# svip-lab/impersonator

Measured on AMD Instinct MI355X. Metric: frames/sec (256x256 motion-imitation, batch=8), higher is better.
Workload: dtype bf16x3; 1 GPU; Imitator inference 256x256 batch=8, random-init ImpersonatorGenerator + synthetic SMPL, 1 source; frames=1024, batch_per_gpu=8, image_size=256, parallelism=frame-sharded replicas x1, grid_sample_align_corners=False, lanes=2, batches_per_launch_sequence=4, frames_per_launch=32, precision=bf16x3, precision_policy=auto

## Files before the change

impersonator_amd/csrc/conv.hip:

```cpp
#include <type_traits>

#include "conv.h"
#include "split.h"
#include "sample.h"

namespace lwg {
namespace {

typedef float f32x16 __attribute__((ext_vector_type(16)));
#pragma clang diagnostic ignored "-Winline-asm"

constexpr int BM = kConvBM;
constexpr int BK = kConvBK;
constexpr int LDK = BK + 4;

template <int BN, int WM, int WN, bool WIDE = false, int NWAVES = 4, int BMT = BM, int TC2 = 0>
__device__ __forceinline__ void igemm_epilogue(const ConvArgs &a, const ConvPhase &ph, int phase, f32x16 (&acc)[WM][WN],
                                               float *smem, int tid, int lane, int wave_m, int wave_n, int img, int rem0, int n0,
                                               int mtile, int sub_stride = 0)
{
    unsigned ones = ~0u;
    asm volatile("" : "+s"(ones));
    lane = (int)__builtin_amdgcn_mbcnt_hi(ones, __builtin_amdgcn_mbcnt_lo(ones, 0u));
    tid = (wave_m * (BN / (32 * WN)) + wave_n) * 64 + lane;
// ... 843 lines not shown
        for (int i = 0; i < WM; ++i)
#pragma unroll
            for (int j = 0; j < WN; ++j)
#pragma unroll
                for (int r = 0; r < 16; ++r) keep += acc[i][j][r];
        if (keep == 123.456f) a.y[0] = 1.f;
    }
    __syncthreads();
    }
}

template <int NHW, int B_CH, int Q, int QB, int NS, int HT = 7>
struct HaloSched {
    static constexpr int nh(int t) { return t < HT ? NHW / HT + (t < NHW % HT ? 1 : 0) : 0; }
    static constexpr int tap_of(int k) { int t = 0; while (hstart(t + 1) <= k) ++t; return t; }
    static constexpr bool dma_at(int t, int q) { for (int p = 0; p < lps(t); ++p) if (pos(t, p) == q) return true; return false; }
    static constexpr int nfree(int t, int q0) { int n = 0; for (int q = q0; q < QB; ++q) n += dma_at(t, q) ? 0 : 1; return n; }
    static constexpr int conv_first(int nconv, int nslot, int slot, int piece) { return conv_range(nconv, nslot, slot, piece) / 16; }
    static constexpr int conv_last(int nconv, int nslot, int slot, int piece) { return conv_range(nconv, nslot, slot, piece) % 16; }
    static constexpr int conv_range(int nconv, int nslot, int slot, int piece) {
        if (nconv == 1) {
            if (piece != 0) return 0;
            if (nslot >= 7)
                return slot == 0 ? 0 * 16 + 1 : slot == 3 ? 1 * 16 + 3 : slot == 4 ? 3 * 16 + 5 : slot == 5 ? 5 * 16 + 7 : slot == 6 ? 7 * 16 + 8 : 0;
            return slot == 0 ? 0 * 16 + 1 : slot == 2 ? 1 * 16 + 4 : slot == 3 ? 4 * 16 + 6 : slot == 4 ? 6 * 16 + 8 : 0;
        }
        if (nslot >= 8) {
            if (slot >= 8 || (slot & 1) != piece) return 0;
            return (slot >> 1) == 0 ? 0 * 16 + 1 : (slot >> 1) == 1 ? 1 * 16 + 3 : (slot >> 1) == 2 ? 3 * 16 + 5 : 5 * 16 + 8;
        }
// ... 9 lines not shown
    }
    static constexpr int hstart(int t) { int n = 0; for (int u = 0; u < t; ++u) n += nh(u); return n; }
    static constexpr int lps(int t) { return nh(t) + B_CH; }
    static constexpr int pos(int t, int p) { return (p + 1) * Q / lps(t) - 1; }
    static constexpr int issued(int t) { int n = 0; for (int p = 0; p < lps(t); ++p) n += pos(t, p) < QB ? 1 : 0; return n; }
    static constexpr int nwait(int t) { int n = issued(t); for (int d = 1; d <= NS - 3; ++d) n += lps((t + 9 - d) % 9); return n; }
};

struct HaloCT {
    static constexpr int phase(int t) { return t == 0 ? 0 : t < 3 ? 1 : t < 5 ? 2 : 3; }
    static constexpr int tap(int t) { return t == 0 ? 0 : t < 3 ? t - 1 : t < 5 ? t - 3 : t - 5; }
    static constexpr int dy(int t) { return (t == 4 || t == 7 || t == 8) ? 1 : 0; }
    static constexpr int dx(int t) { return (t == 2 || t == 6 || t == 8) ? 1 : 0; }
};

template <int BN, int WM, int WN, int NS, int TC, int BMT = BM, int CT = 0, bool RAW = false>
__global__ __launch_bounds__(64 * (BMT / (32 * WM)) * (BN / (32 * WN))) void conv3x3_halo_bf16x3(const ConvArgs a)
{
    constexpr int NPH = CT ? 4 : 1, PADL = CT ? 0 : 1;
    constexpr int WAVES_N = BN / (32 * WN), WAVES_M = BMT / (32 * WM), NW = WAVES_M * WAVES_N;
    static_assert((NW == 4 || NW == 8) && (NS == 3 || NS == 4) && BMT % TC == 0 && TC % 32 == 0, "layout");
    constexpr int TR = BMT / TC, HC = TC + 2 - (CT ? 1 : 0), HR = TR + 2 - (CT ? 1 : 0), HP = HR * HC;
    constexpr int NCH = (HP + 7) / 8;
    constexpr int NHW = (NCH + NW - 1) / NW;
    constexpr int HALO = NCH * 8 * BK;
    constexpr int B_CH = BN / 8 / NW, BSTAGE = BN * BK, BOFF = 2 * HALO;
    static_assert(B_CH >= 1, "a weight chunk per wave");
    constexpr int TILES = WM * WN, Q = 6 * TILES, QB = Q * 3 / 4, NL = 2 * (WM + WN);
    constexpr int RPM = (NL + (Q - QB) - 1) / (Q - QB);
    constexpr int HT = RAW ? 6 : 7;
    using S = HaloSched<NHW, B_CH, Q, QB, NS, HT>;
    static_assert(S::hstart(9) == NHW && Q >= NHW / HT + 1 + B_CH, "halo pieces fit their taps, one piece per MFMA at most");
    static_assert(!RAW || (NW % 2 == 0 && S::tap_of(NHW - 1) + 3 <= 8), "RAW: chunk parity per wave, conversions end ahead of the barrier of tap 8");
    constexpr int DUMMY = BOFF + NS * BSTAGE;
    constexpr int SSOFF = DUMMY + 8 * BK;

    extern __shared__ __attribute__((aligned(16))) float smem[];
    const int tid = threadIdx.x, lane = tid & 63;
    const int wave = __builtin_amdgcn_readfirstlane(tid >> 6);
    const int wave_m = wave / WAVES_N, wave_n = wave % WAVES_N;
    unsigned long long tr_t0 = 0, tr_rt0 = 0, tr_loop0 = 0, tr_loop1 = 0;
    if (a.trace) {
        tr_t0 = __builtin_amdgcn_s_memtime();
        tr_rt0 = __builtin_amdgcn_s_memrealtime();
    }
    int bx = blockIdx.x;
    const int by = blockIdx.y;
    if (!a.natural_order && (gridDim.x & 7) == 0) bx = (blockIdx.x & 7) * (gridDim.x >> 3) + (blockIdx.x >> 3);
// ... 12 lines not shown
    };
    auto dma16 = [&](unsigned voff, const char *sbase, unsigned lds_byte) {
        asm volatile("s_mov_b32 m0, %2\n\t"
                     "s_nop 0\n\t"
                     "global_load_lds_dwordx4 %0, %1"
                     :
                     : "v"(voff), "s"(sbase), "s"(lds_byte)
                     : "memory", "m0");
    };
    const ConvPhase ph = a.ph[0];
    const int lr = lane >> 3, ls = lane & 7;
    const float *xin = a.x + (size_t)img * a.H * a.W * a.ldx;
    const char *x_base = uniform_ptr(xin);
    const unsigned zoff_b = (unsigned)((const char *)a.zeros - (const char *)xin);

    unsigned hoff[NHW];
    unsigned inside = 0;
#pragma unroll
    for (int j = 0; j < NHW; ++j) {
        int c = wave + NW * j;
        if (c >= NCH) c -= NCH;
        const int p = c * 8 + lr;
        const int hr = p / HC, hc = p - hr * HC;
        const int gh = h0 - PADL + hr, gw = w0 - PADL + hc;
        const bool ok = p < HP && (unsigned)gh < (unsigned)a.H && (unsigned)gw < (unsigned)a.W;
        hoff[j] = ok ? (unsigned)(((gh * a.W + gw) * a.ldx + (ls ^ ((p >> 1) & 7)) * 4) * 4) : zoff_b;
        if (RAW && ok && wave + NW * j < NCH) inside |= 1u << j;
    }
    unsigned wvoff[NPH][B_CH];
#pragma unroll
    for (int pp = 0; pp < NPH; ++pp)
#pragma unroll
        for (int j = 0; j < B_CH; ++j) {
            const int row = (wave * B_CH + j) * 8 + lr;
            wvoff[pp][j] = (unsigned)(((n0 + row) * a.ph[pp].Kpad + (ls ^ ((row >> 1) & 7)) * 4) * 4);
        }
    const char *w_phase[NPH];
#pragma unroll
    for (int pp = 0; pp < NPH; ++pp) w_phase[pp] = uniform_ptr(a.w_split + a.ph[pp].w_off);
    const unsigned cin4 = (unsigned)a.Cin * 4u;
    const int nslices = a.Cin / BK;
    const unsigned wave_b = __builtin_amdgcn_readfirstlane(lds_base + (unsigned)((BOFF + wave * B_CH * 8 * BK) * 4));

    auto halo_piece = [&](int j, int sl, int hs) {
        int c = wave + NW * j;
        unsigned dst = (unsigned)((hs * HALO + c * 8 * BK) * 4);
        if (c >= NCH) {
            c -= NCH;
            dst = RAW ? (unsigned)(DUMMY * 4) : (unsigned)((hs * HALO + c * 8 * BK) * 4);
        }
        dma16(hoff[j], x_base + __builtin_amdgcn_readfirstlane((unsigned)sl * (BK * 4u)), __builtin_amdgcn_readfirstlane(lds_base + dst));
    };
    [[maybe_unused]] float4 ssa = {0.f, 0.f, 0.f, 0.f}, ssb = {0.f, 0.f, 0.f, 0.f};
    [[maybe_unused]] auto load_ss = [&](int sl) {
        const int g = ls ^ ((((wave & 1) << 2) + (lr >> 1)) & 7);
        const float *q = smem + SSOFF + (sl * BK - a.raw_from + 4 * g) * 2;
        ssa = *reinterpret_cast<const float4 *>(q);
        ssb = *reinterpret_cast<const float4 *>(q + 4);
    };
    [[maybe_unused]] const int cv_swz = (((wave & 1) << 2) + (lr >> 1)) & 7, cv_g = ls ^ cv_swz;
    [[maybe_unused]] const int cv_rd = lr * 128 + ls * 16;
    [[maybe_unused]] const int cv_hi = lr * 128 + (((cv_g >> 1) ^ cv_swz) << 4) + ((cv_g & 1) << 3);
    [[maybe_unused]] const int cv_lo = lr * 128 + (((4 + (cv_g >> 1)) ^ cv_swz) << 4) + ((cv_g & 1) << 3);
    [[maybe_unused]] const int cv_dummy = DUMMY * 4 + lane * 16;
    struct Conv { float4 v, y, hf; bf16x4_t h, l; int ahi, alo; };
    [[maybe_unused]] Conv cvA, cvB;
    [[maybe_unused]] auto convert_step = [&](int j, Conv &c, int hs, int step, bool live) {
// ... 11 lines not shown
            c.h[0] = (__bf16)c.y.x; c.h[1] = (__bf16)c.y.y; c.h[2] = (__bf16)c.y.z; c.h[3] = (__bf16)c.y.w;
        } else if (step == 4) {
            c.hf = make_float4((float)c.h[0], (float)c.h[1], (float)c.h[2], (float)c.h[3]);
        } else if (step == 5) {
            c.l[0] = (__bf16)(c.y.x - c.hf.x); c.l[1] = (__bf16)(c.y.y - c.hf.y);
            c.l[2] = (__bf16)(c.y.z - c.hf.z); c.l[3] = (__bf16)(c.y.w - c.hf.w);
        } else if (step == 6) {
            c.ahi = live ? chunk + cv_hi : cv_dummy;
            c.alo = live ? chunk + cv_lo : cv_dummy + 8;
        } else {
            *reinterpret_cast<bf16x4_t *>(base + c.ahi) = c.h;
            *reinterpret_cast<bf16x4_t *>(base + c.alo) = c.l;
        }
    };
    auto weight_piece = [&](int jb, int it, int is, int slot) {
        const int pp = CT ? HaloCT::phase(it) : 0, ti = CT ? HaloCT::tap(it) : it;
        dma16(wvoff[pp][jb], w_phase[pp] + __builtin_amdgcn_readfirstlane((unsigned)ti * cin4 + (unsigned)is * (BK * 4u)),
              __builtin_amdgcn_readfirstlane(wave_b + (unsigned)((slot * BSTAGE + jb * 8 * BK) * 4)));
    };

    f32x16 acc[NPH][WM][WN];
#pragma unroll
    for (int pp = 0; pp < NPH; ++pp)
#pragma unroll
        for (int i = 0; i < WM; ++i)
#pragma unroll
            for (int j = 0; j < WN; ++j)
#pragma unroll
                for (int r = 0; r < 16; ++r) acc[pp][i][j][r] = 0.f;

    const int frow = lane & 31, half = lane >> 5, fsw = (frow >> 1) & 7;
    int pl[WM];
#pragma unroll
    for (int i = 0; i < WM; ++i) {
        const int m = wave_m * 32 * WM + i * 32;
        pl[i] = (m / TC) * HC + (m % TC) + frow;
    }
    auto a_addr = [&](int i, int tap, int hs) {
        const int p = pl[i] + (CT ? HaloCT::dy(tap) * HC + HaloCT::dx(tap) : (tap / 3) * HC + (tap % 3));
        return hs * (HALO * 4) + p * 128 + ((half ^ ((p >> 1) & 7)) << 4);
    };
    const int b_row = (wave_n * 32 * WN + frow) * BK;
    int fcol[4];
#pragma unroll
    for (int c = 0; c < 4; ++c) fcol[c] = (((2 * c + half) ^ fsw) * 4);
    struct Frags { float4 ah[WM], al[WM], bh[WN], bl[WN]; };
    const char *smem_b = reinterpret_cast<const char *>(smem);
    auto load_one = [&](const int (&aa)[WM], int bslot, int kb, Frags &f, int idx) {
        const float *Bs = smem + BOFF + bslot * BSTAGE + b_row;
        if (idx < WM) f.al[idx] = *reinterpret_cast<const float4 *>(smem_b + (aa[idx] ^ (64 + 32 * kb)));
        else if (idx < WM + WN) f.bh[idx - WM] = *reinterpret_cast<const float4 *>(Bs + (idx - WM) * 32 * BK + fcol[kb]);
        else if (idx < 2 * WM + WN) f.ah[idx - WM - WN] = *reinterpret_cast<const float4 *>(smem_b + (aa[idx - WM - WN] ^ (32 * kb)));
        else f.bl[idx - 2 * WM - WN] = *reinterpret_cast<const float4 *>(Bs + (idx - 2 * WM - WN) * 32 * BK + fcol[2 + kb]);
    };
    Frags fr;
    int cur_a[WM];

    auto stage_body = [&](auto tap_c, auto issue_c, int sl, int slot) {
        constexpr int T = decltype(tap_c)::value;
        constexpr bool ISSUE = decltype(issue_c)::value;
        constexpr int TN = (T + 1) % 9;
        constexpr int IT = (T + NS - 1) % 9;
        const int slot1 = slot + 1 == NS ? 0 : slot + 1;
        const int slot2 = slot == 0 ? NS - 1 : slot - 1;
        const int hs = sl & 1, hs_next = T == 8 ? hs ^ 1 : hs;
        const int is = sl + (T + NS - 1 >= 9 ? 1 : 0);
        const int sl_halo = sl + 1 < nslices ? sl + 1 : 0;
        Frags f1, nx;
        int nxt_a[WM];
        [[maybe_unused]] const bool raw_next = RAW && sl + 1 < nslices && (sl + 1) * BK >= a.raw_from;
        [[maybe_unused]] const unsigned live_bits = raw_next ? inside : 0u;
        if constexpr (RAW) {
            if (T == S::tap_of(0) + 3) load_ss(sl + 1 < nslices ? sl + 1 : 0);
        }
#pragma unroll
        for (int q = 0; q < Q; ++q) {
            const int kb = q / (3 * TILES), r = q % (3 * TILES);
            const int t = r / TILES, i = (r / WN) % WM, j = r % WN;
            if (q == QB) {
                __builtin_amdgcn_sched_barrier(0);
                if (ISSUE) {
                    asm volatile("s_waitcnt vmcnt(%0) lgkmcnt(0)" ::"n"(S::nwait(T)) : "memory");
                } else {
                    asm volatile("s_waitcnt vmcnt(0) lgkmcnt(0)" ::: "memory");
                }
                __builtin_amdgcn_s_barrier();
                asm volatile("" ::: "memory");
#pragma unroll
                for (int ii = 0; ii < WM; ++ii) nxt_a[ii] = a_addr(ii, TN, hs_next);
            }
            const Frags &f = kb == 0 ? fr : f1;
            const float4 a4 = t == 0 ? f.al[i] : f.ah[i];
            const float4 b4 = t == 1 ? f.bl[j] : f.bh[j];
            constexpr int PP = CT ? HaloCT::phase(T) : 0;
            acc[PP][i][j] = __builtin_amdgcn_mfma_f32_32x32x16_bf16(__builtin_bit_cast(bf16x8_t, a4),
                                                                    __builtin_bit_cast(bf16x8_t, b4), acc[PP][i][j], 0, 0, 0);
            if (q < NL) {
                load_one(cur_a, slot, 1, f1, q);
                __builtin_amdgcn_sched_group_barrier(0x008, 1, 0);
                __builtin_amdgcn_sched_group_barrier(0x100, 1, 0);
            } else if (q >= QB && RPM * (q - QB) < NL) {
#pragma unroll
                for (int r2 = 0; r2 < RPM; ++r2)
                    if (RPM * (q - QB) + r2 < NL) load_one(nxt_a, slot1, 0, nx, RPM * (q - QB) + r2);
                __builtin_amdgcn_sched_group_barrier(0x008, 1, 0);
                __builtin_amdgcn_sched_group_barrier(0x100, RPM, 0);
            }
            if constexpr (RAW) {
                constexpr int NCONV = T >= 3 ? S::nh(T - 3) : 0, K0 = T >= 3 ? S::hstart(T - 3) : 0;
// ... 9 lines not shown
#pragma unroll
                        for (int m = 0; m < 8; ++m)
                            if (m >= a0 && m < a1) convert_step(K0, cvA, hs ^ 1, m, (live_bits >> K0) & 1u);
#pragma unroll
                        for (int m = 0; m < 8; ++m)
                            if (m >= b0 && m < b1) convert_step(K0 + 1, cvB, hs ^ 1, m, (live_bits >> (K0 + 1)) & 1u);
                        __builtin_amdgcn_sched_barrier(0);
                    }
                }
            }
            if (ISSUE) {
#pragma unroll
                for (int p = 0; p < S::lps(T); ++p)
                    if (q == S::pos(T, p)) {
                        __builtin_amdgcn_sched_barrier(0);
                        if (p < S::nh(T)) halo_piece(S::hstart(T) + p, sl_halo, hs ^ 1);
                        else weight_piece(p - S::nh(T), IT, is, slot2);
                        __builtin_amdgcn_sched_barrier(0);
                    }
            }
        }
        fr = nx;
#pragma unroll
        for (int ii = 0; ii < WM; ++ii) cur_a[ii] = nxt_a[ii];
    };

    if constexpr (RAW) {
        const float2 *ss = a.in_ss + (size_t)img * a.in_ss_ld;
        const int nraw = a.Cin - a.raw_from;
        for (int i2 = tid; i2 < nraw; i2 += NW * 64) reinterpret_cast<float2 *>(smem + SSOFF)[i2] = ss[i2];
        asm volatile("s_waitcnt vmcnt(0)" ::: "memory");
    }
#pragma unroll
    for (int j = 0; j < NHW; ++j) halo_piece(j, 0, 0);
#pragma unroll
    for (int st = 0; st < NS - 1; ++st)
#pragma unroll
        for (int jb = 0; jb < B_CH; ++jb) weight_piece(jb, st, 0, st);
    asm volatile("s_waitcnt vmcnt(%0)" ::"n"((NS - 2) * B_CH) : "memory");
    if constexpr (RAW) {
        if (a.raw_from == 0) {
            asm volatile("s_waitcnt lgkmcnt(0)" ::: "memory");
            __builtin_amdgcn_s_barrier();
            asm volatile("" ::: "memory");
            load_ss(0);
#pragma unroll
            for (int j = 0; j < NHW; ++j)
#pragma unroll
                for (int step = 0; step < 8; ++step) convert_step(j, cvA, 0, step, (inside >> j) & 1u);
            asm volatile("s_waitcnt lgkmcnt(0)" ::: "memory");
        }
    }
    __builtin_amdgcn_s_barrier();
    asm volatile("" ::: "memory");
#pragma unroll
    for (int ii = 0; ii < WM; ++ii) cur_a[ii] = a_addr(ii, 0, 0);
#pragma unroll
    for (int idx = 0; idx < NL; ++idx) load_one(cur_a, 0, 0, fr, idx);

    using yes = std::integral_constant<bool, true>;
    using no = std::integral_constant<bool, false>;
    if (a.trace) tr_loop0 = __builtin_amdgcn_s_memtime();
    int slot = 0;
    auto bump = [&]() { slot = slot + 1 == NS ? 0 : slot + 1; };
#define LWG_HALO_STAGE(T, ISS) stage_body(std::integral_constant<int, T>{}, ISS{}, sl, slot); bump();
    for (int sl = 0; sl + 1 < nslices; ++sl) {
        LWG_HALO_STAGE(0, yes) LWG_HALO_STAGE(1, yes) LWG_HALO_STAGE(2, yes) LWG_HALO_STAGE(3, yes) LWG_HALO_STAGE(4, yes)
        LWG_HALO_STAGE(5, yes) LWG_HALO_STAGE(6, yes) LWG_HALO_STAGE(7, yes) LWG_HALO_STAGE(8, yes)
    }
    {
        const int sl = nslices - 1;
        LWG_HALO_STAGE(0, yes) LWG_HALO_STAGE(1, yes) LWG_HALO_STAGE(2, yes) LWG_HALO_STAGE(3, yes) LWG_HALO_STAGE(4, yes)
        LWG_HALO_STAGE(5, yes)
        if constexpr (NS == 3) { LWG_HALO_STAGE(6, yes) } else { LWG_HALO_STAGE(6, no) }
        LWG_HALO_STAGE(7, no) LWG_HALO_STAGE(8, no)
    }
#undef LWG_HALO_STAGE

    if (a.trace) tr_loop1 = __builtin_amdgcn_s_memtime();
    __syncthreads();
    const int part0 = img * (tiles_x * (a.Hm / 4)) + (h0 / 4) * tiles_x + (w0 / TC);
#pragma unroll
    for (int pp = 0; pp < NPH; ++pp) {
// ... 333 lines not shown
}

static bool halo3x3_shape(const ConvArgs &a)
{
    const ConvPhase &p0 = a.ph[0];
    return a.nphase == 1 && p0.KH == 3 && p0.KW == 3 && a.stride == 1 && a.pad == 1 && a.dil == 1 && a.os == 1 && a.H == a.Hm &&
           a.W == a.Wm && p0.Kpad == 9 * a.Cin && a.Wm % 32 == 0 && a.Hm % 4 == 0;
}
static bool haloCT_shape(const ConvArgs &a)
{
    return a.nphase == 4 && a.os == 2 && a.stride == 1 && a.pad == 0 && a.dil == 1 && a.H == a.Hm && a.W == a.Wm && a.Wm % 32 == 0 &&
           a.Hm % 4 == 0 && a.Cout % 64 == 0 && a.ph[0].KH == 1 && a.ph[0].KW == 1 && a.ph[1].KH == 1 && a.ph[1].KW == 2 &&
           a.ph[2].KH == 2 && a.ph[2].KW == 1 && a.ph[3].KH == 2 && a.ph[3].KW == 2 && a.ph[0].Kpad == a.Cin &&
           a.ph[1].Kpad == 2 * a.Cin && a.ph[2].Kpad == 2 * a.Cin && a.ph[3].Kpad == 4 * a.Cin;
}
bool conv_raw_input_supported(const ConvArgs &a, int bn)
{
    static const char *halo_env = getenv("LWG_HALO"), *fused_env = getenv("LWG_FUSED_APPLY");
    if ((halo_env && halo_env[0] == '0') || (fused_env && fused_env[0] == '0')) return false;
    if (a.precision != 1 || a.general || !a.w_split || (a.ldx & 31) || (a.Cin & 31) || a.Cin < 32 || (bn != 64 && bn != 128)) return false;
    if (a.raw_from < 0 || (a.raw_from & 31) || a.raw_from >= a.Cin || a.Cin - a.raw_from > 512) return false;
    return halo3x3_shape(a) || haloCT_shape(a);
}

int launch_conv_igemm(const ConvArgs &a_in, int bn, hipStream_t st, int *variant)
{
    ConvArgs a = a_in;
    a.trace = nullptr;
    const bool bn32_ok = bn == 32 && a.precision == 0 && !a.general && a.Cin >= BK && a.zeros;
    if (a.Cout % bn != 0 || (bn != 64 && bn != 128 && !bn32_ok))
        LWG_FAIL(LWG_ERR_UNSUPPORTED, "conv: Cout=%d not a multiple of the %d-channel tile", a.Cout, bn);
    if (!a.general && ((a.Hm * a.Wm) % BM != 0 || a.mtiles * BM != a.N * a.Hm * a.Wm))
        LWG_FAIL(LWG_ERR_UNSUPPORTED, "conv: %dx%d output grid per image is not a multiple of %d pixels", a.Hm, a.Wm, BM);
    if (a.general && (a.partials || a.fuse_phases || (a.precision != 0 && a.precision != 1) ||
                      a.mtiles != ceil_div((long)a.N * a.Hm * a.Wm, BM)))
        LWG_FAIL(LWG_ERR_INVALID_ARG, "conv: general mode is unfused, without statistics, mtiles = ceil(M/128)");
    if (a.ksplit > 1 && (!a.general || !a.kpart || a.kpart_stride < (size_t)a.N * a.Ho * a.Wo * a.ldy))
        LWG_FAIL(LWG_ERR_INVALID_ARG, "conv: a reduction split needs the general mode and a partial buffer of ksplit outputs");
    if (a.dil < 1) LWG_FAIL(LWG_ERR_INVALID_ARG, "conv: dilation must be >= 1");
    if ((1 << a.cin_log2) != a.Cin || a.Cin < 4 || (a.ldx & 3))
        LWG_FAIL(LWG_ERR_UNSUPPORTED, "conv: Cin=%d must be a power of two >= 4 with a 16-byte aligned pixel stride", a.Cin);
    for (int p = 0; p < a.nphase; ++p)
        if (a.ph[p].Kpad % BK != 0 || a.ph[p].Kpad < a.ph[p].ntaps * a.Cin)
            LWG_FAIL(LWG_ERR_UNSUPPORTED, "conv: bad padded K=%d for %d taps x %d channels", a.ph[p].Kpad, a.ph[p].ntaps, a.Cin);
    if (a.precision == 1 && a.tap_inner)
        for (int p = 0; p < a.nphase; ++p)
            if (a.ph[p].Kpad != a.ph[p].ntaps * a.Cin)
                LWG_FAIL(LWG_ERR_UNSUPPORTED, "conv: taps-innermost walk needs K=%d == %d taps x %d channels", a.ph[p].Kpad,
                         a.ph[p].ntaps, a.Cin);
    if (a.raw_in && (!a.in_ss || !conv_raw_input_supported(a, bn)))
        LWG_FAIL(LWG_ERR_UNSUPPORTED, "conv: raw (un-normalised) input is only taken by the halo-resident bf16x3 kernels");
    const dim3 grid(a.mtiles, a.Cout / bn, a.fuse_phases ? 1 : a.nphase * (a.ksplit > 1 ? a.ksplit : 1));
    const size_t lds = (size_t)2 * (BM + bn) * LDK * sizeof(float);
    static DeviceOnce lds_opt_in;
    if (!lds_opt_in.done()) {
// ... 55 lines not shown
            for (int p = 0; p < a.nphase; ++p)
                if ((size_t)a.Cout * a.ph[p].Kpad * 4 > 0xffffffffull)
                    LWG_FAIL(LWG_ERR_UNSUPPORTED, "conv: weight matrix too large for 32-bit lane offsets");
        }
        const size_t lds3 = (size_t)3 * (BM + bn) * BK * sizeof(float);
        static DeviceOnce opt16;
        if (!opt16.done()) {
            LWG_HIP(hipFuncSetAttribute(reinterpret_cast<const void *>(&conv_igemm_bf16x3<64, 1, 2>),
                                        hipFuncAttributeMaxDynamicSharedMemorySize, 3 * (BM + 64) * BK * (int)sizeof(float)));
            LWG_HIP(hipFuncSetAttribute(reinterpret_cast<const void *>(&conv_igemm_bf16x3<128, 2, 2>),
                                        hipFuncAttributeMaxDynamicSharedMemorySize, 3 * (BM + 128) * BK * (int)sizeof(float)));
            opt16.mark();
        }
        for (int p = 0; p < a.nphase; ++p)
            if (a.ph[p].ntaps > 32) LWG_FAIL(LWG_ERR_UNSUPPORTED, "conv: more than 32 taps on the bf16x3 path");
        static const char *halo_env = getenv("LWG_HALO");
        if (!(halo_env && halo_env[0] == '0') && halo3x3_shape(a)) {
            const int tc = 32;
            static DeviceOnce halo_opt[8];
            const size_t raw_bytes = a.raw_in ? (size_t)8 * BK * sizeof(float) + (size_t)(a.Cin - a.raw_from) * sizeof(float2) : 0;
            auto run = [&](auto kern, int ns, int bmt, DeviceOnce &once) -> int {
                const int hp = (bmt / tc + 2) * (tc + 2), nch = (hp + 7) / 8;
                const size_t base = ((size_t)2 * nch * 8 * BK + (size_t)ns * bn * BK) * sizeof(float), bytes = base + raw_bytes;
                if (!once.done()) {
                    const size_t most = base + (a.raw_in ? (size_t)8 * BK * sizeof(float) + 512 * sizeof(float2) : 0);
                    LWG_HIP(hipFuncSetAttribute(reinterpret_cast<const void *>(kern), hipFuncAttributeMaxDynamicSharedMemorySize, (int)most));
                    once.mark();
                }
                const dim3 g(grid.x / (bmt / BM), grid.y, 1);
                a.trace = trace_block(a, g.x, g.y, bmt == 256 ? 8 : 4, 9 * a.Cin / BK);
                kern<<<g, bmt == 256 ? 512 : 256, bytes, st>>>(a);
// ... 47 lines not shown
                    ct_opt[0].mark();
                }
                kern<<<g, 256, bytes, st>>>(a);
            } else {
                auto kern = &conv3x3_halo_bf16x3<64, 1, 2, 3, 32, 128, 1>;
                if (!ct_opt[1].done()) {
                    LWG_HIP(hipFuncSetAttribute(reinterpret_cast<const void *>(kern), hipFuncAttributeMaxDynamicSharedMemorySize, (int)bytes));
                    ct_opt[1].mark();
                }
                kern<<<g, 256, bytes, st>>>(a);
            }
            if (variant) *variant = wide ? kHaloBf16x3_128 : kHaloBf16x3_64;
            LWG_LAUNCH_CHECK("conv3x3_halo_bf16x3 (transposed)");
            return LWG_OK;
        }
        static const char *ring = getenv("LWG_RING");
        const bool ring4 = !(ring && ring[0] == '3');
        if (g_trace.buf && bn == 128 && ring4) {
            const size_t need = (size_t)grid.x * grid.y * grid.z * 4 * 8 * sizeof(unsigned long long);
            if (g_trace.used + need <= g_trace.bytes && g_trace.n < kTraceMaxLaunches) {
                ConvArgs t = a;
                t.trace = reinterpret_cast<unsigned long long *>(static_cast<char *>(g_trace.buf) + g_trace.used);
                TraceLaunch &L = g_trace.launch[g_trace.n++];
                L.offset = g_trace.used; L.gx = grid.x; L.gy = grid.y; L.gz = grid.z; L.waves = 4;
                L.stages = a.ph[a.fuse_phases ? 0 : 0].Kpad / BK; L.cin = a.Cin; L.cout = a.Cout; L.hm = a.Hm; L.n = a.N;
                g_trace.used += need;
                static DeviceOnce optt;
                if (!optt.done()) {
                    LWG_HIP(hipFuncSetAttribute(reinterpret_cast<const void *>(&conv_igemm_bf16x3<128, 2, 2, 4, 512>),
                                                hipFuncAttributeMaxDynamicSharedMemorySize, 4 * (BM + 128) * BK * (int)sizeof(float)));
                    optt.mark();
                }
                conv_igemm_bf16x3<128, 2, 2, 4, 512><<<grid, 256, (size_t)4 * (BM + 128) * BK * sizeof(float), st>>>(t);
                if (variant) *variant = kIgemmBf16x3_128;
                LWG_LAUNCH_CHECK("conv_igemm_bf16x3 (traced)");
                return LWG_OK;
            }
        }
        static const char *tall_ring_env = getenv("LWG_RING_TALL");
        if (bn == 128 && !a.fuse_phases && a.nphase == 1 && (a.mtiles & 1) == 0 && (a.Hm * a.Wm) % 256 == 0 && !g_trace.buf &&
            (long)(a.mtiles / 2) * (a.Cout / 128) >= device_cu_count() && !(tall_ring_env && tall_ring_env[0] == '0')) {
            static DeviceOnce opt_tall;
            const size_t lds_t = (size_t)3 * (256 + 128) * BK * sizeof(float);
            if (!opt_tall.done()) {
                LWG_HIP(hipFuncSetAttribute(reinterpret_cast<const void *>(&conv_igemm_bf16x3<128, 2, 2, 3, 0, 256>),
                                            hipFuncAttributeMaxDynamicSharedMemorySize, (int)lds_t));
                opt_tall.mark();
            }
            conv_igemm_bf16x3<128, 2, 2, 3, 0, 256><<<dim3(grid.x / 2, grid.y, 1), 512, lds_t, st>>>(a);
            if (variant) *variant = kIgemmBf16x3_128;
            LWG_LAUNCH_CHECK("conv_igemm_bf16x3 (256-row tiles)");
            return LWG_OK;
        }
        if (bn == 64) {
            conv_igemm_bf16x3<64, 1, 2><<<grid, 256, lds3, st>>>(a);
#ifdef LWG_EXPERIMENTS
// ... 255 lines not shown
```

impersonator_amd/csrc/train.hip:

```cpp
#include <algorithm>
#include <cmath>
#include <cstring>
#include <string>
#include <vector>

#include "conv.h"
#include "split.h"
#include "sample.h"

namespace lwg {
namespace {

typedef float f32x16 __attribute__((ext_vector_type(16)));
constexpr float kLeaky = 0.2f;
constexpr float kEps = 1e-5f;

__device__ __forceinline__ float4 ld4(const float *p) { return *reinterpret_cast<const float4 *>(p); }

constexpr int RS_CH = 16, RS_SL = 16;
__global__ __launch_bounds__(256) void in_stats_kernel(const float *__restrict__ x, int HW, int C, float2 *__restrict__ out)
{
    __shared__ double sh[2][RS_SL][RS_CH];
    const int cl = threadIdx.x & (RS_CH - 1), c = blockIdx.x * RS_CH + cl, slice = threadIdx.x / RS_CH, n = blockIdx.y;
    const float *p = x + (size_t)n * HW * C + c;
// ... 1982 lines not shown
        const AdamStep h = {d->step, pow((double)beta1, (double)d->step), pow((double)beta2, (double)d->step)};
        LWG_HIP(hipMemcpy(d->step_dev, &h, sizeof(h), hipMemcpyHostToDevice));
    } else if (d->device_step) {
        AdamStep h;
        LWG_HIP(hipMemcpy(&h, d->step_dev, sizeof(h), hipMemcpyDeviceToHost));
        d->step = h.step;
    }
    d->device_step = on != 0;
    return LWG_OK;
}

namespace {

struct ConvGeom { int Ho, Wo; size_t w_floats; };

int conv_geom(const lwg_conv2d_desc *d, ConvGeom *g)
{
    LWG_REQUIRE(d && g, "conv2d: NULL descriptor");
    auto pow2 = [](int v) { return v > 0 && (v & (v - 1)) == 0; };
    if (!pow2(d->Cin) || !pow2(d->Cout) || d->Cin < 8 || d->Cout < 8)
        LWG_FAIL(LWG_ERR_UNSUPPORTED, "conv2d: channel counts must be powers of two >= 8 (Cin=%d, Cout=%d)", d->Cin, d->Cout);
    if (d->transposed) {
        if (d->k != 3 || d->stride != 2 || d->pad != 1)
            LWG_FAIL(LWG_ERR_UNSUPPORTED, "conv2d: transposed convs are ConvTranspose2d(k3, s2, p1, output_padding 1)");
        g->Ho = 2 * d->H; g->Wo = 2 * d->W;
    } else {
        if (d->stride != 1 && d->stride != 2) LWG_FAIL(LWG_ERR_UNSUPPORTED, "conv2d: stride must be 1 or 2");
        if (d->k < 1 || d->k > 7) LWG_FAIL(LWG_ERR_UNSUPPORTED, "conv2d: kernel size 1..7");
        g->Ho = (d->H + 2 * d->pad - d->k) / d->stride + 1;
        g->Wo = (d->W + 2 * d->pad - d->k) / d->stride + 1;
    }
    if (d->N < 1 || g->Ho < 1 || g->Wo < 1) LWG_FAIL(LWG_ERR_INVALID_ARG, "conv2d: empty tensor");
    g->w_floats = (size_t)d->Cin * d->Cout * d->k * d->k;
    return LWG_OK;
}
// ... 140 lines not shown
SplitWs carve_split(const lwg_conv2d_desc *d, const ConvGeom &g, void *ws)
{
    SplitWs sw;
    float *p = reinterpret_cast<float *>(align_up((size_t)(uintptr_t)ws, (size_t)128)) + base_ws_floats(d, g);
    sw.w = p;
    sw.x = p + align_up(g.w_floats, (size_t)32);
    sw.zeros = sw.x + operand_floats(d, g);
    sw.zero_floats = zero_run_floats(d);
    return sw;
}
}

size_t lwg_conv2d_workspace_bytes(const lwg_conv2d_desc *d)
{
    ConvGeom g;
    if (conv_geom(d, &g) != LWG_OK) return 0;
    size_t floats = base_ws_floats(d, g);
    if (d->precision == 1) floats += align_up(g.w_floats, (size_t)32) + operand_floats(d, g) + zero_run_floats(d) + 32;
    return floats * sizeof(float);
}

int lwg_conv2d_forward(const lwg_conv2d_desc *d, const float *x, const float *w, const float *bias, float *y, void *ws,
                       size_t ws_bytes, lwg_stream_t stream)
{
    ConvGeom g;
    int rc = conv_geom(d, &g);
    if (rc != LWG_OK) return rc;
    LWG_REQUIRE(x && w && y && ws, "conv2d_forward: NULL argument");
    if (ws_bytes < lwg_conv2d_workspace_bytes(d)) LWG_FAIL(LWG_ERR_INVALID_ARG, "conv2d_forward: workspace too small");
    hipStream_t st = reinterpret_cast<hipStream_t>(stream);
    float *wm = static_cast<float *>(ws);
    SplitWs sw_, *sw = nullptr;
    const bool split = d->transposed ? split_route_ok(d->precision, d->Cin, d->H, d->W, 4, nullptr)
                                     : split_route_ok(d->precision, d->Cin, g.Ho, g.Wo, d->k * d->k, bias);
    if (split) { sw_ = carve_split(d, g, ws); sw = &sw_; wm = sw_.w; }
    if (d->transposed) {
        if (bias) LWG_FAIL(LWG_ERR_UNSUPPORTED, "conv2d_forward: bias on a transposed conv");
        if ((rc = relayout(w, wm, 2, d->Cin, d->Cout, 9, (long)g.w_floats, st, 0, split)) != LWG_OK) return rc;
        return op_convT(x, d->N, d->H, d->W, d->Cin, wm, d->Cout, y, st, d->precision, sw);
    }
    const int pitch = (int)align_up((size_t)d->k * d->k * d->Cin, kConvBK);
// ... 485 lines not shown
```

Measured before the change: 3715 frames/s.

## Add stride-2 3x3 halo-tiled bf16x3 convolution kernel with four-plane input staging

Extends the halo-tiled 3x3 convolution kernel to stride-2 convolutions by splitting the input tile into four parity planes staged in a three-slot LDS halo ring. A dedicated per-tap issue schedule lets the halo and weight DMAs overlap the MFMA work. Stride-2 encoder convolutions that previously took the generic implicit-GEMM or ring paths now reuse the input halo across all nine taps instead of re-gathering it. It also relaxes the power-of-two channel check for this shape, at the cost of more LDS per block and a complex hand-written schedule.

```diff
diff --git a/impersonator_amd/csrc/conv.hip b/impersonator_amd/csrc/conv.hip
--- a/impersonator_amd/csrc/conv.hip
+++ b/impersonator_amd/csrc/conv.hip
@@ -881,6 +881,8 @@
 struct HaloSched {
     static constexpr int nh(int t) { return t < HT ? NHW / HT + (t < NHW % HT ? 1 : 0) : 0; }
     static constexpr int tap_of(int k) { int t = 0; while (hstart(t + 1) <= k) ++t; return t; }
+    static constexpr int iplane(int) { return 0; }
+    static constexpr int islice(int) { return 1; }
     static constexpr bool dma_at(int t, int q) { for (int p = 0; p < lps(t); ++p) if (pos(t, p) == q) return true; return false; }
     static constexpr int nfree(int t, int q0) { int n = 0; for (int q = q0; q < QB; ++q) n += dma_at(t, q) ? 0 : 1; return n; }
     static constexpr int conv_first(int nconv, int nslot, int slot, int piece) { return conv_range(nconv, nslot, slot, piece) / 16; }
@@ -920,24 +922,100 @@
     static constexpr int dx(int t) { return (t == 2 || t == 6 || t == 8) ? 1 : 0; }
 };
 
+struct HaloS2 {
+    static constexpr int plane(int t) { return t < 4 ? 0 : t < 6 ? 1 : t < 8 ? 2 : 3; }
+    static constexpr int py(int p) { return p < 2 ? 1 : 0; }
+    static constexpr int px(int p) { return (p & 1) ? 0 : 1; }
+    static constexpr int kh(int t) { const int v[9] = {0, 0, 2, 2, 0, 2, 1, 1, 1}; return v[t]; }
+    static constexpr int kw(int t) { const int v[9] = {0, 2, 0, 2, 1, 1, 0, 2, 1}; return v[t]; }
+    static constexpr int dy(int t) { return (t == 2 || t == 3 || t == 5) ? 1 : 0; }
+    static constexpr int dx(int t) { return (t == 1 || t == 3 || t == 7) ? 1 : 0; }
+    static constexpr bool valid() {
+        for (int k = 0; k < 9; ++k) {
+            int n = 0;
+            for (int t = 0; t < 9; ++t) n += (kh(t) * 3 + kw(t) == k) ? 1 : 0;
+            if (n != 1) return false;
+        }
+        for (int t = 0; t < 9; ++t) {
+            const int p = plane(t);
+            if (dy(t) > py(p) || dx(t) > px(p)) return false;
+            if (2 * dy(t) - py(p) != kh(t) - 1 || 2 * dx(t) - px(p) != kw(t) - 1) return false;
+            if (t && plane(t) < plane(t - 1)) return false;
+        }
+        return true;
+    }
+};
+static_assert(HaloS2::valid(), "stride-2 (plane, tap) tables");
+
+template <int NHW, int B_CH, int Q, int QB, int NS>
+struct HaloSchedS2 {
+    static_assert(NHW == 6, "the table below is for six pieces per wave and plane");
+    static constexpr int nh(int t) { return (t < 2 || t == 8) ? 2 : 3; }
+    static constexpr int iplane(int t) { return t < 2 ? 1 : t < 4 ? 2 : t < 6 ? 3 : t < 8 ? 0 : 1; }
+    static constexpr int islice(int t) { return t >= 6 ? 1 : 0; }
+    static constexpr int hstart(int t) { const int v[9] = {2, 4, 0, 3, 0, 3, 0, 3, 0}; return v[t]; }
+    static constexpr int lps(int t) { return nh(t) + B_CH; }
+    static constexpr int pos(int t, int p) { return (p + 1) * Q / lps(t) - 1; }
+    static constexpr int issued(int t) { int n = 0; for (int p = 0; p < lps(t); ++p) n += pos(t, p) < QB ? 1 : 0; return n; }
+    static constexpr int nwait(int t) {
+        const int next = HaloS2::plane((t + 1) % 9);
+        const bool new_plane = next != HaloS2::plane(t);
+        int n = 0;
+        for (int d = 0; d < 9; ++d) {
+            const int u = (t + 9 - d) % 9;
+            for (int p = lps(u) - 1; p >= 0; --p) {
+                if (d == 0 && pos(u, p) >= QB) continue;
+                const bool weight = p >= nh(u);
+                if (weight ? d == NS - 2 : (new_plane && iplane(u) == next)) return n;
+                ++n;
+            }
+        }
+        return n;
+    }
+    static constexpr bool valid() {
+        bool got[4][NHW] = {};
+        for (int t = 0; t < 9; ++t) {
+            const int ahead = 4 * islice(t) + iplane(t) - HaloS2::plane(t);
+            if (ahead != 1 && ahead != 2) return false;
+            if (ahead == 1 && (t == 8 || HaloS2::plane(t + 1) != HaloS2::plane(t))) return false;
+            for (int k = hstart(t); k < hstart(t) + nh(t); ++k) {
+                if (k >= NHW || got[iplane(t)][k]) return false;
+                got[iplane(t)][k] = true;
+            }
+            if (lps(t) > Q) return false;
+        }
+        for (int p = 0; p < 4; ++p)
+            for (int k = 0; k < NHW; ++k)
+                if (!got[p][k]) return false;
+        return iplane(8) == 1 && islice(8) == 1 && hstart(8) == 0 && iplane(7) == 0 && iplane(6) == 0;
+    }
+};
+
 template <int BN, int WM, int WN, int NS, int TC, int BMT = BM, int CT = 0, bool RAW = false>
 __global__ __launch_bounds__(64 * (BMT / (32 * WM)) * (BN / (32 * WN))) void conv3x3_halo_bf16x3(const ConvArgs a)
 {
-    constexpr int NPH = CT ? 4 : 1, PADL = CT ? 0 : 1;
+    constexpr bool S2 = CT == 2;
+    static_assert(CT >= 0 && CT <= 2 && !(S2 && RAW), "CT: 0 stride 1, 1 transposed, 2 stride 2 (split input only)");
+    constexpr int NPH = CT == 1 ? 4 : 1, PADL = CT ? 0 : 1;
+    constexpr int NPL = S2 ? 4 : 1, NHS = S2 ? 3 : 2;
     constexpr int WAVES_N = BN / (32 * WN), WAVES_M = BMT / (32 * WM), NW = WAVES_M * WAVES_N;
     static_assert((NW == 4 || NW == 8) && (NS == 3 || NS == 4) && BMT % TC == 0 && TC % 32 == 0, "layout");
     constexpr int TR = BMT / TC, HC = TC + 2 - (CT ? 1 : 0), HR = TR + 2 - (CT ? 1 : 0), HP = HR * HC;
     constexpr int NCH = (HP + 7) / 8;
     constexpr int NHW = (NCH + NW - 1) / NW;
     constexpr int HALO = NCH * 8 * BK;
-    constexpr int B_CH = BN / 8 / NW, BSTAGE = BN * BK, BOFF = 2 * HALO;
+    constexpr int B_CH = BN / 8 / NW, BSTAGE = BN * BK, BOFF = NHS * HALO;
     static_assert(B_CH >= 1, "a weight chunk per wave");
     constexpr int TILES = WM * WN, Q = 6 * TILES, QB = Q * 3 / 4, NL = 2 * (WM + WN);
     constexpr int RPM = (NL + (Q - QB) - 1) / (Q - QB);
     constexpr int HT = RAW ? 6 : 7;
-    using S = HaloSched<NHW, B_CH, Q, QB, NS, HT>;
-    static_assert(S::hstart(9) == NHW && Q >= NHW / HT + 1 + B_CH, "halo pieces fit their taps, one piece per MFMA at most");
-    static_assert(!RAW || (NW % 2 == 0 && S::tap_of(NHW - 1) + 3 <= 8), "RAW: chunk parity per wave, conversions end ahead of the barrier of tap 8");
+    using S = std::conditional_t<S2, HaloSchedS2<S2 ? NHW : 6, B_CH, Q, QB, NS>, HaloSched<NHW, B_CH, Q, QB, NS, HT>>;
+    if constexpr (S2) {
+        static_assert(NW == 4 && S::valid(), "stride 2: every piece issued once, into a free slot, ahead of the wait that publishes it");
+    } else {
+        static_assert(S::hstart(9) == NHW && Q >= NHW / HT + 1 + B_CH, "halo pieces fit their taps, one piece per MFMA at most");
+        static_assert(!RAW || (NW % 2 == 0 && S::tap_of(NHW - 1) + 3 <= 8), "RAW: chunk parity per wave, conversions end ahead of the barrier of tap 8");
+    }
     constexpr int DUMMY = BOFF + NS * BSTAGE;
     constexpr int SSOFF = DUMMY + 8 * BK;
 
@@ -980,7 +1058,7 @@
     const char *x_base = uniform_ptr(xin);
     const unsigned zoff_b = (unsigned)((const char *)a.zeros - (const char *)xin);
 
-    unsigned hoff[NHW];
+    unsigned hoff[NPL][NHW];
     unsigned inside = 0;
 #pragma unroll
     for (int j = 0; j < NHW; ++j) {
@@ -988,10 +1066,20 @@
         if (c >= NCH) c -= NCH;
         const int p = c * 8 + lr;
         const int hr = p / HC, hc = p - hr * HC;
-        const int gh = h0 - PADL + hr, gw = w0 - PADL + hc;
-        const bool ok = p < HP && (unsigned)gh < (unsigned)a.H && (unsigned)gw < (unsigned)a.W;
-        hoff[j] = ok ? (unsigned)(((gh * a.W + gw) * a.ldx + (ls ^ ((p >> 1) & 7)) * 4) * 4) : zoff_b;
-        if (RAW && ok && wave + NW * j < NCH) inside |= 1u << j;
+        if constexpr (S2) {
+#pragma unroll
+            for (int pl = 0; pl < NPL; ++pl) {
+                const int py = HaloS2::py(pl), px = HaloS2::px(pl);
+                const int gh = 2 * (h0 + hr) - py, gw = 2 * (w0 + hc) - px;
+                const bool ok = p < HP && (py || hr < TR) && (px || hc < TC) && (unsigned)gh < (unsigned)a.H && (unsigned)gw < (unsigned)a.W;
+                hoff[pl][j] = ok ? (unsigned)(((gh * a.W + gw) * a.ldx + (ls ^ ((p >> 1) & 7)) * 4) * 4) : zoff_b;
+            }
+        } else {
+            const int gh = h0 - PADL + hr, gw = w0 - PADL + hc;
+            const bool ok = p < HP && (unsigned)gh < (unsigned)a.H && (unsigned)gw < (unsigned)a.W;
+            hoff[0][j] = ok ? (unsigned)(((gh * a.W + gw) * a.ldx + (ls ^ ((p >> 1) & 7)) * 4) * 4) : zoff_b;
+            if (RAW && ok && wave + NW * j < NCH) inside |= 1u << j;
+        }
     }
     unsigned wvoff[NPH][B_CH];
 #pragma unroll
@@ -1008,15 +1096,16 @@
     const int nslices = a.Cin / BK;
     const unsigned wave_b = __builtin_amdgcn_readfirstlane(lds_base + (unsigned)((BOFF + wave * B_CH * 8 * BK) * 4));
 
-    auto halo_piece = [&](int j, int sl, int hs) {
+    auto halo_piece = [&](int j, int sl, int hs, int pl = 0) {
         int c = wave + NW * j;
         unsigned dst = (unsigned)((hs * HALO + c * 8 * BK) * 4);
         if (c >= NCH) {
             c -= NCH;
             dst = RAW ? (unsigned)(DUMMY * 4) : (unsigned)((hs * HALO + c * 8 * BK) * 4);
         }
-        dma16(hoff[j], x_base + __builtin_amdgcn_readfirstlane((unsigned)sl * (BK * 4u)), __builtin_amdgcn_readfirstlane(lds_base + dst));
-    };
+        dma16(hoff[pl][j], x_base + __builtin_amdgcn_readfirstlane((unsigned)sl * (BK * 4u)), __builtin_amdgcn_readfirstlane(lds_base + dst));
+    };
+    [[maybe_unused]] auto slot3 = [](int s3, int pl) { const int u = s3 + pl; return u >= 6 ? u - 6 : u >= 3 ? u - 3 : u; };
     [[maybe_unused]] float4 ssa = {0.f, 0.f, 0.f, 0.f}, ssb = {0.f, 0.f, 0.f, 0.f};
     [[maybe_unused]] auto load_ss = [&](int sl) {
         const int g = ls ^ ((((wave & 1) << 2) + (lr >> 1)) & 7);
@@ -1058,7 +1147,7 @@
         }
     };
     auto weight_piece = [&](int jb, int it, int is, int slot) {
-        const int pp = CT ? HaloCT::phase(it) : 0, ti = CT ? HaloCT::tap(it) : it;
+        const int pp = CT == 1 ? HaloCT::phase(it) : 0, ti = CT == 1 ? HaloCT::tap(it) : S2 ? HaloS2::kh(it) * 3 + HaloS2::kw(it) : it;
         dma16(wvoff[pp][jb], w_phase[pp] + __builtin_amdgcn_readfirstlane((unsigned)ti * cin4 + (unsigned)is * (BK * 4u)),
               __builtin_amdgcn_readfirstlane(wave_b + (unsigned)((slot * BSTAGE + jb * 8 * BK) * 4)));
     };
@@ -1081,7 +1170,9 @@
         pl[i] = (m / TC) * HC + (m % TC) + frow;
     }
     auto a_addr = [&](int i, int tap, int hs) {
-        const int p = pl[i] + (CT ? HaloCT::dy(tap) * HC + HaloCT::dx(tap) : (tap / 3) * HC + (tap % 3));
+        const int p = pl[i] + (CT == 1 ? HaloCT::dy(tap) * HC + HaloCT::dx(tap)
+                               : S2    ? HaloS2::dy(tap) * HC + HaloS2::dx(tap)
+                                       : (tap / 3) * HC + (tap % 3));
         return hs * (HALO * 4) + p * 128 + ((half ^ ((p >> 1) & 7)) << 4);
     };
     const int b_row = (wave_n * 32 * WN + frow) * BK;
@@ -1099,6 +1190,7 @@
     };
     Frags fr;
     int cur_a[WM];
+    [[maybe_unused]] int sl3 = 0;
 
     auto stage_body = [&](auto tap_c, auto issue_c, int sl, int slot) {
         constexpr int T = decltype(tap_c)::value;
@@ -1107,9 +1199,12 @@
         constexpr int IT = (T + NS - 1) % 9;
         const int slot1 = slot + 1 == NS ? 0 : slot + 1;
         const int slot2 = slot == 0 ? NS - 1 : slot - 1;
-        const int hs = sl & 1, hs_next = T == 8 ? hs ^ 1 : hs;
+        const int hs = S2 ? slot3(sl3, HaloS2::plane(T)) : sl & 1;
+        const int hs_next = S2 ? slot3(sl3 + (T == 8 ? 1 : 0), HaloS2::plane(TN)) : T == 8 ? hs ^ 1 : hs;
         const int is = sl + (T + NS - 1 >= 9 ? 1 : 0);
-        const int sl_halo = sl + 1 < nslices ? sl + 1 : 0;
+        const int sl_next = sl + S::islice(T);
+        const int sl_halo = sl_next < nslices ? sl_next : 0;
+        auto hs_issue = [&]() { return S2 ? slot3(sl3 + S::islice(T), S::iplane(T)) : hs ^ 1; };
         Frags f1, nx;
         int nxt_a[WM];
         [[maybe_unused]] const bool raw_next = RAW && sl + 1 < nslices && (sl + 1) * BK >= a.raw_from;
@@ -1136,7 +1231,7 @@
             const Frags &f = kb == 0 ? fr : f1;
             const float4 a4 = t == 0 ? f.al[i] : f.ah[i];
             const float4 b4 = t == 1 ? f.bl[j] : f.bh[j];
-            constexpr int PP = CT ? HaloCT::phase(T) : 0;
+            constexpr int PP = CT == 1 ? HaloCT::phase(T) : 0;
             acc[PP][i][j] = __builtin_amdgcn_mfma_f32_32x32x16_bf16(__builtin_bit_cast(bf16x8_t, a4),
                                                                     __builtin_bit_cast(bf16x8_t, b4), acc[PP][i][j], 0, 0, 0);
             if (q < NL) {
@@ -1176,7 +1271,7 @@
                 for (int p = 0; p < S::lps(T); ++p)
                     if (q == S::pos(T, p)) {
                         __builtin_amdgcn_sched_barrier(0);
-                        if (p < S::nh(T)) halo_piece(S::hstart(T) + p, sl_halo, hs ^ 1);
+                        if (p < S::nh(T)) halo_piece(S::hstart(T) + p, sl_halo, hs_issue(), S::iplane(T));
                         else weight_piece(p - S::nh(T), IT, is, slot2);
                         __builtin_amdgcn_sched_barrier(0);
                     }
@@ -1193,6 +1288,19 @@
         for (int i2 = tid; i2 < nraw; i2 += NW * 64) reinterpret_cast<float2 *>(smem + SSOFF)[i2] = ss[i2];
         asm volatile("s_waitcnt vmcnt(0)" ::: "memory");
     }
+    if constexpr (S2) {
+#pragma unroll
+        for (int j = 0; j < NHW; ++j) halo_piece(j, 0, slot3(0, 0), 0);
+#pragma unroll
+        for (int st = 0; st < NS - 2; ++st)
+#pragma unroll
+            for (int jb = 0; jb < B_CH; ++jb) weight_piece(jb, st, 0, st);
+#pragma unroll
+        for (int j = 0; j < S::nh(8); ++j) halo_piece(j, 0, slot3(0, 1), 1);
+#pragma unroll
+        for (int jb = 0; jb < B_CH; ++jb) weight_piece(jb, NS - 2, 0, NS - 2);
+        asm volatile("s_waitcnt vmcnt(%0)" ::"n"((NS - 2) * B_CH + S::nh(8)) : "memory");
+    } else {
 #pragma unroll
     for (int j = 0; j < NHW; ++j) halo_piece(j, 0, 0);
 #pragma unroll
@@ -1200,6 +1308,7 @@
 #pragma unroll
         for (int jb = 0; jb < B_CH; ++jb) weight_piece(jb, st, 0, st);
     asm volatile("s_waitcnt vmcnt(%0)" ::"n"((NS - 2) * B_CH) : "memory");
+    }
     if constexpr (RAW) {
         if (a.raw_from == 0) {
             asm volatile("s_waitcnt lgkmcnt(0)" ::: "memory");
@@ -1229,6 +1338,7 @@
     for (int sl = 0; sl + 1 < nslices; ++sl) {
         LWG_HALO_STAGE(0, yes) LWG_HALO_STAGE(1, yes) LWG_HALO_STAGE(2, yes) LWG_HALO_STAGE(3, yes) LWG_HALO_STAGE(4, yes)
         LWG_HALO_STAGE(5, yes) LWG_HALO_STAGE(6, yes) LWG_HALO_STAGE(7, yes) LWG_HALO_STAGE(8, yes)
+        if constexpr (S2) sl3 = sl3 == 2 ? 0 : sl3 + 1;
     }
     {
         const int sl = nslices - 1;
@@ -1592,6 +1702,12 @@
            a.ph[2].KH == 2 && a.ph[2].KW == 1 && a.ph[3].KH == 2 && a.ph[3].KW == 2 && a.ph[0].Kpad == a.Cin &&
            a.ph[1].Kpad == 2 * a.Cin && a.ph[2].Kpad == 2 * a.Cin && a.ph[3].Kpad == 4 * a.Cin;
 }
+static bool haloS2_shape(const ConvArgs &a)
+{
+    const ConvPhase &p0 = a.ph[0];
+    return a.nphase == 1 && p0.KH == 3 && p0.KW == 3 && a.stride == 2 && a.pad == 1 && a.dil == 1 && a.os == 1 && a.H == 2 * a.Hm &&
+           a.W == 2 * a.Wm && a.Wm % 32 == 0 && a.Hm % 4 == 0 && p0.Kpad == 9 * a.Cin && !a.general && !a.bias && !a.raw_in;
+}
 bool conv_raw_input_supported(const ConvArgs &a, int bn)
 {
     static const char *halo_env = getenv("LWG_HALO"), *fused_env = getenv("LWG_FUSED_APPLY");
@@ -1616,7 +1732,15 @@
     if (a.ksplit > 1 && (!a.general || !a.kpart || a.kpart_stride < (size_t)a.N * a.Ho * a.Wo * a.ldy))
         LWG_FAIL(LWG_ERR_INVALID_ARG, "conv: a reduction split needs the general mode and a partial buffer of ksplit outputs");
     if (a.dil < 1) LWG_FAIL(LWG_ERR_INVALID_ARG, "conv: dilation must be >= 1");
-    if ((1 << a.cin_log2) != a.Cin || a.Cin < 4 || (a.ldx & 3))
+    static const char *tall_ring_env = getenv("LWG_RING_TALL");
+    const bool ring_tall = a.precision == 1 && !a.general && bn == 128 && !a.fuse_phases && a.nphase == 1 && (a.mtiles & 1) == 0 &&
+                           (a.Hm * a.Wm) % 256 == 0 && (long)(a.mtiles / 2) * (a.Cout / 128) >= device_cu_count() &&
+                           !(tall_ring_env && tall_ring_env[0] == '0');
+    static const char *halo_env = getenv("LWG_HALO");
+    static const char *halo_s2_env = getenv("LWG_HALO_S2");
+    const bool s2_halo = a.precision == 1 && !(halo_env && halo_env[0] == '0') && !(halo_s2_env && halo_s2_env[0] == '0') &&
+                         haloS2_shape(a) && !ring_tall && !a.partials;
+    if ((!s2_halo && (1 << a.cin_log2) != a.Cin) || a.Cin < 4 || (a.ldx & 3))
         LWG_FAIL(LWG_ERR_UNSUPPORTED, "conv: Cin=%d must be a power of two >= 4 with a 16-byte aligned pixel stride", a.Cin);
     for (int p = 0; p < a.nphase; ++p)
         if (a.ph[p].Kpad % BK != 0 || a.ph[p].Kpad < a.ph[p].ntaps * a.Cin)
@@ -1702,7 +1826,6 @@
         }
         for (int p = 0; p < a.nphase; ++p)
             if (a.ph[p].ntaps > 32) LWG_FAIL(LWG_ERR_UNSUPPORTED, "conv: more than 32 taps on the bf16x3 path");
-        static const char *halo_env = getenv("LWG_HALO");
         if (!(halo_env && halo_env[0] == '0') && halo3x3_shape(a)) {
             const int tc = 32;
             static DeviceOnce halo_opt[8];
@@ -1780,6 +1903,32 @@
             LWG_LAUNCH_CHECK("conv3x3_halo_bf16x3 (transposed)");
             return LWG_OK;
         }
+        if (s2_halo) {
+            const int ns = bn == 128 ? 4 : 3;
+            const int nch = ((4 + 1) * (32 + 1) + 7) / 8;
+            const size_t bytes = ((size_t)3 * nch * 8 * BK + (size_t)ns * bn * BK) * sizeof(float);
+            const dim3 g(a.mtiles, a.Cout / bn, 1);
+            a.trace = trace_block(a, g.x, g.y, 4, 9 * a.Cin / BK);
+            static DeviceOnce s2_opt[2];
+            if (bn == 128) {
+                auto kern = &conv3x3_halo_bf16x3<128, 2, 2, 4, 32, 128, 2>;
+                if (!s2_opt[0].done()) {
+                    LWG_HIP(hipFuncSetAttribute(reinterpret_cast<const void *>(kern), hipFuncAttributeMaxDynamicSharedMemorySize, (int)bytes));
+                    s2_opt[0].mark();
+                }
+                kern<<<g, 256, bytes, st>>>(a);
+            } else {
+                auto kern = &conv3x3_halo_bf16x3<64, 1, 2, 3, 32, 128, 2>;
+                if (!s2_opt[1].done()) {
+                    LWG_HIP(hipFuncSetAttribute(reinterpret_cast<const void *>(kern), hipFuncAttributeMaxDynamicSharedMemorySize, (int)bytes));
+                    s2_opt[1].mark();
+                }
+                kern<<<g, 256, bytes, st>>>(a);
+            }
+            if (variant) *variant = bn == 128 ? kHaloBf16x3_128 : kHaloBf16x3_64;
+            LWG_LAUNCH_CHECK("conv3x3_halo_bf16x3 (stride 2)");
+            return LWG_OK;
+        }
         static const char *ring = getenv("LWG_RING");
         const bool ring4 = !(ring && ring[0] == '3');
         if (g_trace.buf && bn == 128 && ring4) {
@@ -1803,9 +1952,7 @@
                 return LWG_OK;
             }
         }
-        static const char *tall_ring_env = getenv("LWG_RING_TALL");
-        if (bn == 128 && !a.fuse_phases && a.nphase == 1 && (a.mtiles & 1) == 0 && (a.Hm * a.Wm) % 256 == 0 && !g_trace.buf &&
-            (long)(a.mtiles / 2) * (a.Cout / 128) >= device_cu_count() && !(tall_ring_env && tall_ring_env[0] == '0')) {
+        if (ring_tall && !g_trace.buf) {
             static DeviceOnce opt_tall;
             const size_t lds_t = (size_t)3 * (256 + 128) * BK * sizeof(float);
             if (!opt_tall.done()) {
diff --git a/impersonator_amd/csrc/train.hip b/impersonator_amd/csrc/train.hip
--- a/impersonator_amd/csrc/train.hip
+++ b/impersonator_amd/csrc/train.hip
@@ -2020,11 +2020,13 @@
 
 struct ConvGeom { int Ho, Wo; size_t w_floats; };
 
-int conv_geom(const lwg_conv2d_desc *d, ConvGeom *g)
+int conv_geom(const lwg_conv2d_desc *d, ConvGeom *g, bool forward = false)
 {
     LWG_REQUIRE(d && g, "conv2d: NULL descriptor");
     auto pow2 = [](int v) { return v > 0 && (v & (v - 1)) == 0; };
-    if (!pow2(d->Cin) || !pow2(d->Cout) || d->Cin < 8 || d->Cout < 8)
+    const bool s2_halo = forward && d->precision == 1 && !d->transposed && d->k == 3 && d->stride == 2 && d->pad == 1 &&
+                         d->Cin >= 32 && d->Cin % 32 == 0 && d->Cout >= 64 && d->Cout % 64 == 0 && d->H % 8 == 0 && d->W % 64 == 0;
+    if (!s2_halo && (!pow2(d->Cin) || !pow2(d->Cout) || d->Cin < 8 || d->Cout < 8))
         LWG_FAIL(LWG_ERR_UNSUPPORTED, "conv2d: channel counts must be powers of two >= 8 (Cin=%d, Cout=%d)", d->Cin, d->Cout);
     if (d->transposed) {
         if (d->k != 3 || d->stride != 2 || d->pad != 1)
@@ -2195,7 +2197,7 @@
 size_t lwg_conv2d_workspace_bytes(const lwg_conv2d_desc *d)
 {
     ConvGeom g;
-    if (conv_geom(d, &g) != LWG_OK) return 0;
+    if (conv_geom(d, &g, true) != LWG_OK) return 0;
     size_t floats = base_ws_floats(d, g);
     if (d->precision == 1) floats += align_up(g.w_floats, (size_t)32) + operand_floats(d, g) + zero_run_floats(d) + 32;
     return floats * sizeof(float);
@@ -2205,7 +2207,7 @@
                        size_t ws_bytes, lwg_stream_t stream)
 {
     ConvGeom g;
-    int rc = conv_geom(d, &g);
+    int rc = conv_geom(d, &g, true);
     if (rc != LWG_OK) return rc;
     LWG_REQUIRE(x && w && y && ws, "conv2d_forward: NULL argument");
     if (ws_bytes < lwg_conv2d_workspace_bytes(d)) LWG_FAIL(LWG_ERR_INVALID_ARG, "conv2d_forward: workspace too small");
```

Result: no change. 3713 frames/s (-0.1%).
